# Y-Claw/Multilevel-GNN

Measured on AMD Instinct MI355X. Metric: graphs/sec fwd+bwd, 3-level GNN on 10k-node d=128 synthetic; HBM GB/s %peak, higher is better.
Workload: dtype f32; 1 GPU; configs[1]: ER graphs N=10000 E=160000 x64 per GPU, d=128, 3 GENConv(softmax, res+, LayerNorm) + projection pooling G=25000 k=2 + DiffPool 146->37->10, fp32; step = CSR build (of the next batch, on a second stream) + fwd + bwd + grad all-reduce + Adam; graphs_per_gpu=64, global_batch=64, parallelism=dp1, world_size=1, allreduce_bytes=1429768

## Files before the change

multilevel-gnn_amd/csrc/linear_bwd.hip:

```cpp
#include "split_precision.h"
#include "launch.h"
#include "mlgnn.h"

namespace mlgnn {

constexpr int kLbThreads = 512, kLbWaves = 8, kLbStage = 32;
enum { LB_LN = 0, LB_PLAIN = 1, LB_SHIFT = 2 };

struct LbArgs {
  const float* go; const float* w; const float* x;
  const float* go_parts; const float* x_parts;
  float* dx; float* ws; float* out_parts;
  const float* rstd; const float* gamma; const float* beta;
  const float* lse; float* gt; int* spread;
  int N; int slab_cols;
  int parts_max_with_old;
};

template <int OFF>
__device__ __forceinline__ float lds_read_f32(uint32_t addr) {
  float v;
  asm volatile("ds_read_b32 %0, %1 offset:%2" : "=v"(v) : "v"(addr), "n"(OFF));
  return v;
}
template <int OFF>
__device__ __forceinline__ i32x4 lds_read_b128(uint32_t addr) {
  i32x4 v;
  asm volatile("ds_read_b128 %0, %1 offset:%2" : "=v"(v) : "v"(addr), "n"(OFF));
  return v;
}
template <int OFF>
__device__ __forceinline__ i32x2 lds_read_tr16(uint32_t addr) {
  i32x2 v;
  asm volatile("ds_read_b64_tr_b16 %0, %1 offset:%2" : "=v"(v) : "v"(addr), "n"(OFF));
  return v;
}
#define LB_WAIT_LGKM(N) asm volatile("s_waitcnt lgkmcnt(" #N ")" ::: "memory")
template <int N>
__device__ __forceinline__ void lgkm_landed(i32x4& a, i32x4& b) {
  asm volatile("s_waitcnt lgkmcnt(%2)" : "+v"(a), "+v"(b) : "n"(N) : "memory");
}
template <int N>
__device__ __forceinline__ void lgkm_landed(i32x4& a, i32x4& b, i32x4& c, i32x4& d) {
  asm volatile("s_waitcnt lgkmcnt(%4)" : "+v"(a), "+v"(b), "+v"(c), "+v"(d) : "n"(N) : "memory");
}
template <int N>
__device__ __forceinline__ void lgkm_landed(i32x2& a, i32x2& b, i32x2& c, i32x2& d) {
  asm volatile("s_waitcnt lgkmcnt(%4)" : "+v"(a), "+v"(b), "+v"(c), "+v"(d) : "n"(N) : "memory");
}
template <int N>
__device__ __forceinline__ void lgkm_landed(float (&x)[8]) {
  asm volatile("s_waitcnt lgkmcnt(%8)"
               : "+v"(x[0]), "+v"(x[1]), "+v"(x[2]), "+v"(x[3]), "+v"(x[4]), "+v"(x[5]), "+v"(x[6]), "+v"(x[7])
               : "n"(N) : "memory");
}
template <int N>
__device__ __forceinline__ void lgkm_landed(float (&x)[16]) {
  asm volatile("s_waitcnt lgkmcnt(%16)"
               : "+v"(x[0]), "+v"(x[1]), "+v"(x[2]), "+v"(x[3]), "+v"(x[4]), "+v"(x[5]), "+v"(x[6]), "+v"(x[7]),
                 "+v"(x[8]), "+v"(x[9]), "+v"(x[10]), "+v"(x[11]), "+v"(x[12]), "+v"(x[13]), "+v"(x[14]), "+v"(x[15])
               : "n"(N) : "memory");
}
template <int N>
__device__ __forceinline__ void vm_landed(float (&x)[8]) {
  asm volatile("s_waitcnt vmcnt(%8)"
               : "+v"(x[0]), "+v"(x[1]), "+v"(x[2]), "+v"(x[3]), "+v"(x[4]), "+v"(x[5]), "+v"(x[6]), "+v"(x[7])
               : "n"(N) : "memory");
}
template <int IMM>
__device__ __forceinline__ float glb_load_f32(const void* base, uint32_t byte_off) {
  float v;
  asm volatile("global_load_dword %0, %1, %2 offset:%3" : "=v"(v) : "v"(byte_off), "s"(base), "n"(IMM));
  return v;
}
template <int N>
__device__ __forceinline__ void lb_wait_vm() {
  static_assert(N >= 0 && N <= 63, "vmcnt is a 6-bit counter");
  asm volatile("s_waitcnt vmcnt(%0)" ::"n"(N) : "memory");
}


template <int M, int K, int EPI>
__global__ __launch_bounds__(kLbThreads) void linear_bwd_kernel(const LbArgs p) {
  constexpr int NC = K / 32, NM = kLbWaves / NC, MW = M / NM;
  static_assert(NC * NM == kLbWaves && MW == 128, "instantiated for (M, K) = (128, 256) and (256, 128)");
  static_assert(EPI != LB_LN || NM == 1, "the LayerNorm epilogue needs the whole m range in one wave");
  constexpr int KS = MW / 16;
  constexpr int MT = MW / 32;
  constexpr int GS = M + 4;
  constexpr int kPlaneB = 4 * GS * 16;
  constexpr int kBufB = 2 * kPlaneB;
  constexpr int kXStageB = kLbStage * K * 4;
  constexpr int UPT = M * 4 / kLbThreads;
  constexpr int DMA = kXStageB / 1024 / kLbWaves;
  constexpr int kExB = 2 * kBufB + 3 * kXStageB;
  constexpr int kTotOff = 4 * M + 64;
  constexpr int kExFloats = 4 * M + 64 + (NM == 2 ? kLbWaves * 512 : kLbWaves * 64);
  constexpr int kRsB = kExB + kExFloats * 4;
  extern __shared__ __attribute__((aligned(1024))) unsigned char smem[];
  const uint32_t lds0 = (uint32_t)(uintptr_t)smem;
  float* ex = reinterpret_cast<float*>(smem + kExB);

  const int tid = threadIdx.x;
  const int lane = tid & (kWave - 1);
  const int wave = __builtin_amdgcn_readfirstlane(tid >> 6);
  const int r31 = lane & 31, h = lane >> 5;
  const int c = wave % NC, mh = wave / NC;
  const int col = 32 * c + r31;

  const int n_stages = (p.N + kLbStage - 1) / kLbStage;
  const int s_begin = (int)((int64_t)n_stages * blockIdx.x / gridDim.x);
  const int s_end = (int)((int64_t)n_stages * (blockIdx.x + 1) / gridDim.x);
  const int n = s_end - s_begin;

  float sa, ia, sx, ix, sw, iw;
  pow2_scale(fold_max_parts(p.go_parts), sa, ia);
  pow2_scale(fold_max_parts(p.x_parts), sx, ix);
  {
    float m = 0.f;
    for (int i = tid; i < M * K / 4; i += kLbThreads) {
      const float4 q = reinterpret_cast<const float4*>(p.w)[i];
      m = fmaxf(m, fmaxf(fmaxf(fabsf(q.x), fabsf(q.y)), fmaxf(fabsf(q.z), fabsf(q.w))));
    }
    m = wave_max(m);
    if (lane == 0) ex[wave] = m;
    __syncthreads();
    m = ex[0];
#pragma unroll
    for (int i = 1; i < kLbWaves; ++i) m = fmaxf(m, ex[i]);
    pow2_scale(m, sw, iw);
    __syncthreads();
  }
  auto uniform = [](float v) { return __builtin_bit_cast(float, __builtin_amdgcn_readfirstlane(__builtin_bit_cast(int, v))); };
  sa = uniform(sa); sx = uniform(sx); sw = uniform(sw);
  const float ux = uniform(ia * iw), uw = uniform(ia * ix);

  f16x8 wh[KS], wl[KS];
#pragma unroll
  for (int s = 0; s < KS; ++s) {
    float v[8];
#pragma unroll
    for (int j = 0; j < 8; ++j) v[j] = p.w[(size_t)(mh * MW + 16 * s + 8 * h + j) * K + col];
    split2(v, sw, wh[s], wl[s]);
  }
  float gam = 0.f, bet = 0.f;
  if constexpr (EPI == LB_LN) { gam = p.gamma[col]; bet = p.beta[col]; }
  const bool shift = EPI != LB_SHIFT || p.gt != nullptr;

  auto ucol = [&](int q) { return (tid + q * kLbThreads) % M; };
  auto ubase = [&](int q) { const int G = (tid + q * kLbThreads) / M; return 16 * (G >> 1) + 4 * (G & 1); };
  uint32_t ulds[UPT], goff[UPT];
#pragma unroll
  for (int q = 0; q < UPT; ++q) {
    ulds[q] = (uint32_t)(((tid + q * kLbThreads) / M) * GS + ucol(q)) * 16u;
    goff[q] = (uint32_t)(ubase(q) * M + ucol(q)) * 4u;
  }
  float gr[UPT][8];
  float bsum[UPT];
#pragma unroll
  for (int q = 0; q < UPT; ++q) bsum[q] = 0.f;

  auto row_of = [&](int i) { return (s_begin + min(i, n - 1)) * kLbStage; };
  auto fetch_go = [&](int r0) {
    if (r0 + kLbStage <= p.N) {
      const float* base = p.go + (size_t)r0 * M;
#pragma unroll
      for (int q = 0; q < UPT; ++q) {
        const uint32_t o0 = goff[q], o1 = goff[q] + 8u * M * 4u;
        gr[q][0] = glb_load_f32<0>(base, o0); gr[q][1] = glb_load_f32<M * 4>(base, o0);
        gr[q][2] = glb_load_f32<2 * M * 4>(base, o0); gr[q][3] = glb_load_f32<3 * M * 4>(base, o0);
        gr[q][4] = glb_load_f32<0>(base, o1); gr[q][5] = glb_load_f32<M * 4>(base, o1);
        gr[q][6] = glb_load_f32<2 * M * 4>(base, o1); gr[q][7] = glb_load_f32<3 * M * 4>(base, o1);
      }
    } else {
#pragma unroll
      for (int q = 0; q < UPT; ++q) {
#pragma unroll
        for (int j = 0; j < 8; ++j) {
          const int row = min(r0 + ubase(q) + (j & 3) + 8 * (j >> 2), p.N - 1);
          gr[q][j] = glb_load_f32<0>(p.go, (uint32_t)(row * M + ucol(q)) * 4u);
        }
      }
    }
  };
  auto commit_go = [&](int buf, int r0, bool valid) {
    const bool full = r0 + kLbStage <= p.N;
#pragma unroll
    for (int q = 0; q < UPT; ++q) {
      float v[8];
      float s = 0.f;
#pragma unroll
      for (int j = 0; j < 8; ++j) {
        const bool keep = valid && (full || r0 + ubase(q) + (j & 3) + 8 * (j >> 2) < p.N);
        v[j] = keep ? gr[q][j] : 0.f;
        s += v[j];
      }
      bsum[q] += s;
      f16x8 hi, lo;
      split2(v, sa, hi, lo);
      unsigned char* dst = smem + buf * kBufB + ulds[q];
      *reinterpret_cast<f16x8*>(dst) = hi;
      *reinterpret_cast<f16x8*>(dst + kPlaneB) = lo;
    }
  };
  auto dma_x = [&](int r0, int xbuf) {
#pragma unroll
    for (int i = 0; i < DMA; ++i) {
      const int piece = wave * DMA + i;
      const int e = piece * 256 + lane * 4;
      const int row = min(r0 + e / K, p.N - 1);
      const float* src = p.x + (size_t)row * K + (e % K);
      __builtin_amdgcn_global_load_lds((glb_void_t*)src, (lds_void_t*)(smem + 2 * kBufB + xbuf * kXStageB + piece * 1024), 16, 0, 0);
    }
  };

  f32x16 accw[MT];
#pragma unroll
  for (int t = 0; t < MT; ++t)
#pragma unroll
    for (int r = 0; r < 16; ++r) accw[t][r] = 0.f;
  float dgam = 0.f, dbet = 0.f, om = 0.f, worst = 0.f;

  const uint32_t a_w = lds0 + (uint32_t)((h * GS) + mh * MW + r31) * 16u;
  uint32_t a_tr;
  {
    const int g16 = lane >> 4, b = g16 & 1, hh = g16 >> 1, q = (lane >> 2) & 3, pp = lane & 3;
    a_tr = lds0 + (uint32_t)((2 * b + (pp & 1)) * GS + mh * MW + 8 * hh + q) * 16u + 8u * (uint32_t)(pp >> 1);
  }
  const uint32_t a_x = lds0 + 2 * kBufB + (uint32_t)((4 * h) * K + col) * 4u;

  constexpr int E_L = EPI == LB_LN ? 1 : (EPI == LB_SHIFT ? 8 : 0);
  constexpr int E_S = EPI == LB_SHIFT ? 16 : (EPI == LB_LN ? 16 : 8);
  constexpr int kVmPerIter = E_L + 8 * UPT + DMA + E_S;

  if (n > 0) {
    fetch_go(row_of(0));
    dma_x(row_of(0), 0);
    dma_x(row_of(1), 1);
#pragma unroll
    for (int q = 0; q < UPT; ++q) vm_landed<0>(gr[q]);
    commit_go(0, row_of(0), true);
    __syncthreads();

    for (int i = 0; i < n; ++i) {
      const int r0 = row_of(i);
      const bool full = r0 + kLbStage <= p.N;
      const int buf = i & 1, xbuf = i % 3;
      float lse8[EPI == LB_SHIFT ? 8 : 1];
      if constexpr (EPI == LB_LN) {
        if (lane < 8)
          __builtin_amdgcn_global_load_lds((glb_void_t*)(p.rstd + min(r0 + 4 * lane, (p.N - 1) & ~3)),
                                           (lds_void_t*)(smem + kRsB + ((i % 3) * kLbWaves + wave) * 256), 16, 0, 0);
      }
      if constexpr (EPI == LB_SHIFT) {
        if (!shift) {
#pragma unroll
          for (int q = 0; q < 8; ++q) lse8[q] = glb_load_f32<0>(p.go_parts, 0u);
        } else if (full) {
          const float* base = p.lse + (size_t)r0 * K;
          const uint32_t o0 = (uint32_t)((16 * mh + 4 * h) * K + col) * 4u, o1 = o0 + 8u * K * 4u;
          lse8[0] = glb_load_f32<0>(base, o0); lse8[1] = glb_load_f32<K * 4>(base, o0);
          lse8[2] = glb_load_f32<2 * K * 4>(base, o0); lse8[3] = glb_load_f32<3 * K * 4>(base, o0);
          lse8[4] = glb_load_f32<0>(base, o1); lse8[5] = glb_load_f32<K * 4>(base, o1);
          lse8[6] = glb_load_f32<2 * K * 4>(base, o1); lse8[7] = glb_load_f32<3 * K * 4>(base, o1);
        } else {
#pragma unroll
          for (int q = 0; q < 8; ++q)
            lse8[q] = glb_load_f32<0>(p.lse, (uint32_t)(min(r0 + mfma32_row(8 * mh + q, h), p.N - 1) * K + col) * 4u);
        }
      }
      fetch_go(row_of(i + 1));
      dma_x(row_of(i + 2), (i + 2) % 3);
      __builtin_amdgcn_sched_barrier(0);

      float xv[16];
      {
        const uint32_t ax = a_x + (uint32_t)xbuf * kXStageB;
#define LB_XV(R) xv[R] = lds_read_f32<mfma32_row(R, 0) * K * 4>(ax);
        LB_XV(0) LB_XV(1) LB_XV(2) LB_XV(3) LB_XV(4) LB_XV(5) LB_XV(6) LB_XV(7)
        LB_XV(8) LB_XV(9) LB_XV(10) LB_XV(11) LB_XV(12) LB_XV(13) LB_XV(14) LB_XV(15)
#undef LB_XV
      }
      const uint32_t aw = a_w + (uint32_t)buf * kBufB;
      i32x4 fa[2][2];
      fa[0][0] = lds_read_b128<0>(aw);
      fa[0][1] = lds_read_b128<kPlaneB>(aw);
      lgkm_landed<2>(xv);
#pragma unroll
      for (int kk = 0; kk < 2; ++kk) {
        float v[8];
#pragma unroll
        for (int j = 0; j < 8; ++j) {
          v[j] = xv[8 * kk + j];
          if constexpr (EPI == LB_LN) v[j] = relu_keep_nan(fmaf(v[j], gam, bet));
        }
        f16x8 bh, bl;
        split2(v, sx, bh, bl);
#pragma unroll
        for (int t = 0; t < MT; ++t) {
          const int step = kk * MT + t, slot = step & 1;
          if (step + 1 < 2 * MT) {
            constexpr int kStepB = 2 * GS * 16;
            const int nkk = (step + 1) / MT, nt = (step + 1) % MT;
            if (nkk == 0) {
              if (nt == 1) { fa[1][0] = lds_read_b128<512>(aw); fa[1][1] = lds_read_b128<kPlaneB + 512>(aw); }
              if (nt == 2) { fa[0][0] = lds_read_b128<1024>(aw); fa[0][1] = lds_read_b128<kPlaneB + 1024>(aw); }
              if (nt == 3) { fa[1][0] = lds_read_b128<1536>(aw); fa[1][1] = lds_read_b128<kPlaneB + 1536>(aw); }
            } else {
              if (nt == 0) { fa[0][0] = lds_read_b128<kStepB>(aw); fa[0][1] = lds_read_b128<kPlaneB + kStepB>(aw); }
              if (nt == 1) { fa[1][0] = lds_read_b128<kStepB + 512>(aw); fa[1][1] = lds_read_b128<kPlaneB + kStepB + 512>(aw); }
              if (nt == 2) { fa[0][0] = lds_read_b128<kStepB + 1024>(aw); fa[0][1] = lds_read_b128<kPlaneB + kStepB + 1024>(aw); }
              if (nt == 3) { fa[1][0] = lds_read_b128<kStepB + 1536>(aw); fa[1][1] = lds_read_b128<kPlaneB + kStepB + 1536>(aw); }
            }
            lgkm_landed<2>(fa[slot][0], fa[slot][1]);
          } else {
            lgkm_landed<0>(fa[slot][0], fa[slot][1]);
          }
          const f16x8 ah = __builtin_bit_cast(f16x8, fa[slot][0]), al = __builtin_bit_cast(f16x8, fa[slot][1]);
          f32x16 cw = accw[t];
          cw = __builtin_amdgcn_mfma_f32_32x32x16_f16(al, bh, cw, 0, 0, 0);
          cw = __builtin_amdgcn_mfma_f32_32x32x16_f16(ah, bl, cw, 0, 0, 0);
          cw = __builtin_amdgcn_mfma_f32_32x32x16_f16(ah, bh, cw, 0, 0, 0);
          accw[t] = cw;
        }
      }
      __builtin_amdgcn_sched_barrier(0);
      f32x16 accx;
#pragma unroll
      for (int r = 0; r < 16; ++r) accx[r] = 0.f;
      {
        const uint32_t at = a_tr + (uint32_t)buf * kBufB;
        i32x2 ft[2][4];
#define LB_TR(SLOT, S)                                                                              \
        ft[SLOT][0] = lds_read_tr16<(S) * 256>(at); ft[SLOT][1] = lds_read_tr16<(S) * 256 + 64>(at); \
        ft[SLOT][2] = lds_read_tr16<kPlaneB + (S) * 256>(at); ft[SLOT][3] = lds_read_tr16<kPlaneB + (S) * 256 + 64>(at);
#define LB_DX(SLOT, S)                                                                              \
        {                                                                                           \
          const i32x4 hi4 = {ft[SLOT][0][0], ft[SLOT][0][1], ft[SLOT][1][0], ft[SLOT][1][1]};       \
          const i32x4 lo4 = {ft[SLOT][2][0], ft[SLOT][2][1], ft[SLOT][3][0], ft[SLOT][3][1]};       \
          const f16x8 ah = __builtin_bit_cast(f16x8, hi4), al = __builtin_bit_cast(f16x8, lo4);     \
          accx = __builtin_amdgcn_mfma_f32_32x32x16_f16(al, wh[S], accx, 0, 0, 0);                  \
          accx = __builtin_amdgcn_mfma_f32_32x32x16_f16(ah, wl[S], accx, 0, 0, 0);                  \
          accx = __builtin_amdgcn_mfma_f32_32x32x16_f16(ah, wh[S], accx, 0, 0, 0);                  \
        }
#define LB_LANDED(SLOT, CNT) lgkm_landed<CNT>(ft[SLOT][0], ft[SLOT][1], ft[SLOT][2], ft[SLOT][3]);
        LB_TR(0, 0)
        LB_TR(1, 1) LB_LANDED(0, 4) LB_DX(0, 0)
        LB_TR(0, 2) LB_LANDED(1, 4) LB_DX(1, 1)
        LB_TR(1, 3) LB_LANDED(0, 4) LB_DX(0, 2)
        LB_TR(0, 4) LB_LANDED(1, 4) LB_DX(1, 3)
        LB_TR(1, 5) LB_LANDED(0, 4) LB_DX(0, 4)
        LB_TR(0, 6) LB_LANDED(1, 4) LB_DX(1, 5)
        LB_TR(1, 7) LB_LANDED(0, 4) LB_DX(0, 6)
        LB_LANDED(1, 0) LB_DX(1, 7)
#undef LB_LANDED
#undef LB_TR
#undef LB_DX
      }

      __builtin_amdgcn_sched_barrier(0);
      if constexpr (EPI == LB_LN) {
        float g[16];
        const bool odd_row = (lane & 16) != 0;
        const int r_mine = lane & 15;
        float mine = 0.f;
#pragma unroll
        for (int r = 0; r < 16; ++r) {
          const bool live = full || r0 + mfma32_row(r, h) < p.N;
          const float y = fmaf(xv[r], gam, bet);
          const float gy = (live && y > 0.f) ? accx[r] * ux : 0.f;
          dgam = fmaf(gy, xv[r], dgam);
          dbet += gy;
          g[r] = gy * gam;
          const float gx = g[r] * xv[r];
          const float recv = __builtin_bit_cast(float, __builtin_amdgcn_ds_swizzle(
              __builtin_bit_cast(int, odd_row ? g[r] : gx), 0x401f));
          float u = (odd_row ? gx : g[r]) + recv;
          u += dpp_row_ror<8>(u); u += dpp_row_ror<4>(u); u += dpp_row_ror<2>(u); u += dpp_row_ror<1>(u);
          mine = (r_mine == r) ? u : mine;
        }
        ex[wave * 64 + lane] = mine;
        lb_wait_vm<8 * UPT + DMA>();
        const uint32_t ars = lds0 + kRsB + (uint32_t)(((i % 3) * kLbWaves + wave) * 256 + 16 * h);
        i32x4 rs0_ = lds_read_b128<0>(ars), rs1_ = lds_read_b128<32>(ars), rs2_ = lds_read_b128<64>(ars),
              rs3_ = lds_read_b128<96>(ars);
        lgkm_landed<0>(rs0_, rs1_, rs2_, rs3_);
        float rs[16];
#pragma unroll
        for (int q = 0; q < 4; ++q) {
          rs[q] = __builtin_bit_cast(f32x4, rs0_)[q]; rs[4 + q] = __builtin_bit_cast(f32x4, rs1_)[q];
          rs[8 + q] = __builtin_bit_cast(f32x4, rs2_)[q]; rs[12 + q] = __builtin_bit_cast(f32x4, rs3_)[q];
        }
        __builtin_amdgcn_s_barrier();
        float tot;
        {
          const uint32_t ae = lds0 + kExB + (uint32_t)lane * 4u;
          float e[8] = {lds_read_f32<0>(ae), lds_read_f32<256>(ae), lds_read_f32<512>(ae), lds_read_f32<768>(ae),
                        lds_read_f32<1024>(ae), lds_read_f32<1280>(ae), lds_read_f32<1536>(ae), lds_read_f32<1792>(ae)};
          lgkm_landed<0>(e);
          tot = ((((((e[0] + e[1]) + e[2]) + e[3]) + e[4]) + e[5]) + e[6]) + e[7];
        }
        constexpr float inv_k = 1.0f / K;
#pragma unroll
        for (int r = 0; r < 16; ++r) {
          const float s1 = __shfl(tot, 32 * h + r) * inv_k;
          const float s2 = __shfl(tot, 32 * h + 16 + r) * inv_k;
          g[r] = rs[r] * (g[r] - s1 - xv[r] * s2);
          if (!full && r0 + mfma32_row(r, h) >= p.N) g[r] = 0.f;
          om = fmaxf(om, fabsf(g[r]));
        }
        char* out = reinterpret_cast<char*>(p.dx + (size_t)r0 * K);
        const uint32_t o0 = (uint32_t)(4 * h * K + col) * 4u;
        if (full) {
#pragma unroll
          for (int r = 0; r < 16; ++r)
            *reinterpret_cast<float*>(out + (o0 + (uint32_t)(mfma32_row(r, 0) * K * 4))) = g[r];
        } else {
#pragma unroll
          for (int r = 0; r < 16; ++r)
            if (r0 + mfma32_row(r, h) < p.N)
              *reinterpret_cast<float*>(out + (o0 + (uint32_t)(mfma32_row(r, 0) * K * 4))) = g[r];
        }
      } else {
        float keep[8];
        if constexpr (NM == 2) {
          float* mine = ex + wave * 512 + lane;
#pragma unroll
          for (int q = 0; q < 8; ++q) {
            keep[q] = mh ? accx[8 + q] : accx[q];
            mine[q * 64] = mh ? accx[q] : accx[8 + q];
          }
          LB_WAIT_LGKM(0);
          __builtin_amdgcn_s_barrier();
          const uint32_t ae = lds0 + kExB + (uint32_t)((wave ^ NC) * 512 + lane) * 4u;
          float e[8] = {lds_read_f32<0>(ae), lds_read_f32<256>(ae), lds_read_f32<512>(ae), lds_read_f32<768>(ae),
                        lds_read_f32<1024>(ae), lds_read_f32<1280>(ae), lds_read_f32<1536>(ae), lds_read_f32<1792>(ae)};
          lgkm_landed<0>(e);
#pragma unroll
          for (int q = 0; q < 8; ++q) keep[q] += e[q];
        } else {
#pragma unroll
          for (int q = 0; q < 8; ++q) keep[q] = 0.f;
        }
        if constexpr (EPI == LB_SHIFT) vm_landed<8 * UPT + DMA>(lse8);
        else asm volatile("" : "+v"(keep[0]), "+v"(keep[1]), "+v"(keep[2]), "+v"(keep[3]), "+v"(keep[4]), "+v"(keep[5]),
                          "+v"(keep[6]), "+v"(keep[7])::"memory");
        float v[8], gt[8];
#pragma unroll
        for (int q = 0; q < 8; ++q) {
          v[q] = keep[q] * ux;
          om = fmaxf(om, fabsf(v[q]));
          if constexpr (EPI == LB_SHIFT) {
            gt[q] = v[q] * fast_exp2(-lse8[q]);
            if (shift) worst = fmaxf(worst, fabsf(lse8[q]));
          }
        }
        char* out = reinterpret_cast<char*>(p.dx + (size_t)r0 * K);
        char* out_t = reinterpret_cast<char*>(p.gt + (size_t)r0 * K);
        const uint32_t o0 = (uint32_t)((16 * mh + 4 * h) * K + col) * 4u;
        if (full) {
#pragma unroll
          for (int q = 0; q < 8; ++q)
            *reinterpret_cast<float*>(out + (o0 + (uint32_t)(mfma32_row(q, 0) * K * 4))) = v[q];
          if (EPI == LB_SHIFT && shift) {
#pragma unroll
            for (int q = 0; q < 8; ++q)
              *reinterpret_cast<float*>(out_t + (o0 + (uint32_t)(mfma32_row(q, 0) * K * 4))) = gt[q];
          }
        } else {
#pragma unroll
          for (int q = 0; q < 8; ++q) {
            if (r0 + mfma32_row(8 * mh + q, h) < p.N) {
              const uint32_t o = o0 + (uint32_t)(mfma32_row(q, 0) * K * 4);
              *reinterpret_cast<float*>(out + o) = v[q];
              if (EPI == LB_SHIFT && shift) *reinterpret_cast<float*>(out_t + o) = gt[q];
            }
          }
        }
      }

      __builtin_amdgcn_sched_barrier(0);
      if (full && shift) {
#pragma unroll
        for (int q = 0; q < UPT; ++q) vm_landed<DMA + E_S>(gr[q]);
      } else if (full) {
#pragma unroll
        for (int q = 0; q < UPT; ++q) vm_landed<DMA + (EPI == LB_SHIFT ? 8 : E_S)>(gr[q]);
      } else {
#pragma unroll
        for (int q = 0; q < UPT; ++q) vm_landed<0>(gr[q]);
      }
      commit_go(buf ^ 1, row_of(i + 1), i + 1 < n);
      if (full && shift) lb_wait_vm<kVmPerIter>();
      else if (full) lb_wait_vm<kVmPerIter - (EPI == LB_SHIFT ? 8 : 0)>();
      else lb_wait_vm<0>();
      LB_WAIT_LGKM(0);
      __builtin_amdgcn_s_barrier();
    }
  }
  lb_wait_vm<0>();

  float* slab = p.ws + (size_t)blockIdx.x * p.slab_cols;
#pragma unroll
  for (int t = 0; t < MT; ++t)
#pragma unroll
    for (int r = 0; r < 16; ++r)
      slab[(size_t)(mh * MW + 32 * t + mfma32_row(r, h)) * K + col] = accw[t][r] * uw;
  __syncthreads();
#pragma unroll
  for (int q = 0; q < UPT; ++q) {
    const int u = tid + q * kLbThreads;
    ex[(u / M) * M + ucol(q)] = bsum[q];
  }
  if constexpr (EPI == LB_LN) {
    dgam += __shfl_xor(dgam, 32);
    dbet += __shfl_xor(dbet, 32);
    if (h == 0) { slab[M * K + M + col] = dgam; slab[M * K + M + K + col] = dbet; }
  }
#pragma unroll
  for (int off = 32; off > 0; off >>= 1) { om = fmaxf(om, __shfl_xor(om, off)); worst = fmaxf(worst, __shfl_xor(worst, off)); }
  if (lane == 0) ex[4 * M + wave] = om;
  __syncthreads();
  for (int m = tid; m < M; m += kLbThreads) slab[M * K + m] = (ex[m] + ex[M + m]) + (ex[2 * M + m] + ex[3 * M + m]);
  if (tid == 0 && p.out_parts) {
    float m = ex[4 * M];
#pragma unroll
    for (int i = 1; i < kLbWaves; ++i) m = fmaxf(m, ex[4 * M + i]);
    p.out_parts[blockIdx.x] = p.parts_max_with_old ? fmaxf(m, p.out_parts[blockIdx.x]) : m;
  }
  if constexpr (EPI == LB_SHIFT) {
    if (shift && lane == 0 && worst > kMaxLse) *p.spread = 1;
  }
}

__global__ __launch_bounds__(256) void lb_rowmax_parts_kernel(const float* __restrict__ a, float* __restrict__ pa,
                                                             const float* __restrict__ b, float* __restrict__ pb, int n,
                                                             int* __restrict__ zero4, float* __restrict__ zero_parts) {
  __shared__ float red[2][4];
  if (blockIdx.x == 0 && threadIdx.x < 4 && zero4) zero4[threadIdx.x] = 0;
  if (threadIdx.x == 0 && zero_parts) zero_parts[blockIdx.x] = 0.f;
  const int per = (n + kMaxParts - 1) / kMaxParts;
  const int lo = blockIdx.x * per, hi = min(n, lo + per);
  float ma = 0.f, mb = 0.f;
  for (int i = lo + threadIdx.x; i < hi; i += 256) { if (a) ma = fmaxf(ma, a[i]); if (b) mb = fmaxf(mb, b[i]); }
#pragma unroll
  for (int off = 32; off > 0; off >>= 1) { ma = fmaxf(ma, __shfl_xor(ma, off)); mb = fmaxf(mb, __shfl_xor(mb, off)); }
  if ((threadIdx.x & 63) == 0) { red[0][threadIdx.x >> 6] = ma; red[1][threadIdx.x >> 6] = mb; }
  __syncthreads();
  if (threadIdx.x == 0) {
    if (a) pa[blockIdx.x] = fmaxf(fmaxf(red[0][0], red[0][1]), fmaxf(red[0][2], red[0][3]));
    if (b) pb[blockIdx.x] = fmaxf(fmaxf(red[1][0], red[1][1]), fmaxf(red[1][2], red[1][3]));
  }
}

template <int M, int K>
constexpr int lb_lds_bytes() {
  return 2 * (2 * 4 * (M + 4) * 16) + 3 * (kLbStage * K * 4) + (4 * M + 64) * 4 +
         (M == 256 ? kLbWaves * 512 * 4 : kLbWaves * 64 * 4) +
         3 * kLbWaves * 256;
}

}

using namespace mlgnn;

static bool lb_shape_ok(int64_t N, int64_t M, int64_t K, int epi) {
  if (N <= 0 || N > INT32_MAX - kLbStage) return false;
  if (epi == LB_LN) return M == 128 && K == 256;
  return M == 256 && K == 128;
}

extern "C" int mlgnn_linear_bwd_supported(int64_t N, int64_t M, int64_t K, int epilogue) {
  if (epilogue != LB_LN && epilogue != LB_PLAIN && epilogue != LB_SHIFT) return 0;
  return lb_shape_ok(N, M, K, epilogue) ? 1 : 0;
}

extern "C" int64_t mlgnn_linear_bwd_workspace_floats(int64_t N, int64_t M, int64_t K, int epilogue) {
  if (!mlgnn_linear_bwd_supported(N, M, K, epilogue)) return MLGNN_E_SHAPE;
  const int64_t cols = M * K + M + (epilogue == LB_LN ? 2 * K : 0);
  return (int64_t)kMaxParts * cols + 3 * kMaxParts;
}

extern "C" int mlgnn_linear_bwd(const float* go, const float* w, const float* x, const float* go_max, int go_max_is_parts,
                                const float* x_row_max, int epilogue, const float* rstd, const float* gamma,
                                const float* beta, const float* lse, float* dx, float* grad_shifted,
                                int32_t* shift_flag, float* grad_w_b, float* dx_max_parts, float* workspace,
                                int64_t workspace_floats, int64_t N, int64_t M, int64_t K, void* stream) {
  if (epilogue != LB_LN && epilogue != LB_PLAIN && epilogue != LB_SHIFT) return MLGNN_E_MODE;
  if (!lb_shape_ok(N, M, K, epilogue)) return MLGNN_E_SHAPE;
  if (!go || !w || !x || !go_max || !x_row_max || !dx || !grad_w_b || !workspace) return MLGNN_E_NULL;
  if (epilogue == LB_LN && (!rstd || !gamma || !beta)) return MLGNN_E_NULL;
  if (epilogue == LB_SHIFT && (!lse || !grad_shifted || !shift_flag)) return MLGNN_E_NULL;
  if (workspace_floats < mlgnn_linear_bwd_workspace_floats(N, M, K, epilogue)) return MLGNN_E_WORKSPACE;
  if (!aligned(go, w, x, rstd)) return MLGNN_E_ALIGN;
  hipStream_t s = as_stream(stream);
  const int cols = (int)(M * K + M + (epilogue == LB_LN ? 2 * K : 0));
  float* parts = workspace + (int64_t)kMaxParts * cols;
  const int64_t stages = (N + kLbStage - 1) / kLbStage;
  const int grid = (int)(stages < kMaxParts ? stages : kMaxParts);
  hipLaunchKernelGGL(lb_rowmax_parts_kernel, dim3(kMaxParts), dim3(256), 0, s, go_max_is_parts ? nullptr : go_max, parts,
                     x_row_max, parts + kMaxParts, (int)N, epilogue == LB_SHIFT ? shift_flag : nullptr,
                     (dx_max_parts && grid < kMaxParts) ? dx_max_parts : nullptr);
  int err;
  LbArgs a;
  a.w = w; a.go_parts = go_max_is_parts ? go_max : parts; a.x_parts = parts + kMaxParts;
  a.ws = workspace; a.out_parts = dx_max_parts;
  a.gamma = gamma; a.beta = beta;
  a.spread = shift_flag;
  a.slab_cols = cols;
  const auto launch = [&](auto kernel, int lds_bytes, int grid) {
    if (const hipError_t e = allow_dynamic_lds(kernel, lds_bytes); e != hipSuccess) return (int)e;
    hipLaunchKernelGGL(kernel, dim3(grid), dim3(kLbThreads), lds_bytes, s, a);
    return (int)hipGetLastError();
  };
  if (epilogue == LB_PLAIN) { lse = nullptr; grad_shifted = nullptr; a.spread = nullptr; }
  const int64_t slab_rows = dense_slab_rows(M > K ? M : K);
  for (int64_t r0 = 0; r0 < N; r0 += slab_rows) {
    const int64_t n = N - r0 < slab_rows ? N - r0 : slab_rows;
    const int64_t st = (n + kLbStage - 1) / kLbStage;
    const int grid = (int)(st < kMaxParts ? st : kMaxParts);
    a.go = go + r0 * M; a.x = x + r0 * K; a.dx = dx + r0 * K;
    a.rstd = rstd ? rstd + r0 : nullptr;
    a.lse = lse ? lse + r0 * K : nullptr; a.gt = grad_shifted ? grad_shifted + r0 * K : nullptr;
    a.N = (int)n; a.parts_max_with_old = r0 > 0;
    err = epilogue == LB_LN ? launch(&linear_bwd_kernel<128, 256, LB_LN>, lb_lds_bytes<128, 256>(), grid)
                            : launch(&linear_bwd_kernel<256, 128, LB_SHIFT>, lb_lds_bytes<256, 128>(), grid);
    if (err) return err;
    launch_reduce_partials(workspace, grad_w_b, grid, cols, s, r0 > 0);
  }
  return (int)hipGetLastError();
}
```

Before: 5481 graphs/s.

## Double-buffer LDS exchange area to drop end-of-iteration barrier in linear backward

The cross-wave exchange area in LDS is double-buffered by iteration parity. This lets the trailing vmcnt/lgkmcnt wait and s_barrier at the end of each stage loop be removed, and the commit of the next go tile moves ahead of the epilogue. In the LayerNorm epilogue, the per-row totals are now written back to LDS and read with pipelined ds_read_b64 together with rstd, replacing 32 cross-lane shuffles. The cost is more LDS per block and subtler ordering guarantees between iterations, which rely on the remaining mid-epilogue barrier.

```diff
diff --git a/multilevel-gnn_amd/csrc/linear_bwd.hip b/multilevel-gnn_amd/csrc/linear_bwd.hip
--- a/multilevel-gnn_amd/csrc/linear_bwd.hip
+++ b/multilevel-gnn_amd/csrc/linear_bwd.hip
@@ -4,6 +4,7 @@
 
 namespace mlgnn {
 
+using f32x2 = __attribute__((ext_vector_type(2))) float;
 constexpr int kLbThreads = 512, kLbWaves = 8, kLbStage = 32;
 enum { LB_LN = 0, LB_PLAIN = 1, LB_SHIFT = 2 };
 
@@ -30,19 +31,28 @@
   return v;
 }
 template <int OFF>
+__device__ __forceinline__ i32x2 lds_read_b64(uint32_t addr) {
+  i32x2 v;
+  asm volatile("ds_read_b64 %0, %1 offset:%2" : "=v"(v) : "v"(addr), "n"(OFF));
+  return v;
+}
+template <int OFF>
 __device__ __forceinline__ i32x2 lds_read_tr16(uint32_t addr) {
   i32x2 v;
   asm volatile("ds_read_b64_tr_b16 %0, %1 offset:%2" : "=v"(v) : "v"(addr), "n"(OFF));
   return v;
 }
+__device__ __forceinline__ void lds_write_f32(uint32_t addr, float v) {
+  asm volatile("ds_write_b32 %0, %1" ::"v"(addr), "v"(v) : "memory");
+}
 #define LB_WAIT_LGKM(N) asm volatile("s_waitcnt lgkmcnt(" #N ")" ::: "memory")
 template <int N>
 __device__ __forceinline__ void lgkm_landed(i32x4& a, i32x4& b) {
   asm volatile("s_waitcnt lgkmcnt(%2)" : "+v"(a), "+v"(b) : "n"(N) : "memory");
 }
 template <int N>
-__device__ __forceinline__ void lgkm_landed(i32x4& a, i32x4& b, i32x4& c, i32x4& d) {
-  asm volatile("s_waitcnt lgkmcnt(%4)" : "+v"(a), "+v"(b), "+v"(c), "+v"(d) : "n"(N) : "memory");
+__device__ __forceinline__ void lgkm_landed(i32x2& a, i32x2& b, i32x2& c) {
+  asm volatile("s_waitcnt lgkmcnt(%3)" : "+v"(a), "+v"(b), "+v"(c) : "n"(N) : "memory");
 }
 template <int N>
 __device__ __forceinline__ void lgkm_landed(i32x2& a, i32x2& b, i32x2& c, i32x2& d) {
@@ -79,6 +89,15 @@
   asm volatile("s_waitcnt vmcnt(%0)" ::"n"(N) : "memory");
 }
 
+
+template <int M>
+constexpr int lb_exchange_floats() { return kLbWaves * (M == 256 ? 512 : 64); }
+template <int M, int K>
+constexpr int lb_lds_bytes() {
+  return 2 * (2 * 4 * (M + 4) * 16) + 3 * (kLbStage * K * 4) + 2 * lb_exchange_floats<M>() * 4 +
+         (M == 256 ? 0 : 3 * kLbWaves * 256);
+}
+static_assert(lb_lds_bytes<128, 256>() <= 160 * 1024 && lb_lds_bytes<256, 128>() <= 160 * 1024, "160 KiB of LDS per CU");
 
 template <int M, int K, int EPI>
 __global__ __launch_bounds__(kLbThreads) void linear_bwd_kernel(const LbArgs p) {
@@ -94,9 +113,11 @@
   constexpr int UPT = M * 4 / kLbThreads;
   constexpr int DMA = kXStageB / 1024 / kLbWaves;
   constexpr int kExB = 2 * kBufB + 3 * kXStageB;
-  constexpr int kTotOff = 4 * M + 64;
-  constexpr int kExFloats = 4 * M + 64 + (NM == 2 ? kLbWaves * 512 : kLbWaves * 64);
+  constexpr int kParFloats = lb_exchange_floats<M>();
+  constexpr int kExFloats = 2 * kParFloats;
+  static_assert(kExFloats >= 4 * M + kLbWaves, "the tail of the kernel folds the bias sums and the maxima in this area");
   constexpr int kRsB = kExB + kExFloats * 4;
+  static_assert(kRsB + (EPI == LB_LN ? 3 * kLbWaves * 256 : 0) == lb_lds_bytes<M, K>(), "lb_lds_bytes() is this layout");
   extern __shared__ __attribute__((aligned(1024))) unsigned char smem[];
   const uint32_t lds0 = (uint32_t)(uintptr_t)smem;
   float* ex = reinterpret_cast<float*>(smem + kExB);
@@ -229,9 +250,6 @@
   }
   const uint32_t a_x = lds0 + 2 * kBufB + (uint32_t)((4 * h) * K + col) * 4u;
 
-  constexpr int E_L = EPI == LB_LN ? 1 : (EPI == LB_SHIFT ? 8 : 0);
-  constexpr int E_S = EPI == LB_SHIFT ? 16 : (EPI == LB_LN ? 16 : 8);
-  constexpr int kVmPerIter = E_L + 8 * UPT + DMA + E_S;
 
   if (n > 0) {
     fetch_go(row_of(0));
@@ -359,6 +377,12 @@
       }
 
       __builtin_amdgcn_sched_barrier(0);
+      if constexpr (EPI == LB_SHIFT) vm_landed<DMA>(lse8);
+#pragma unroll
+      for (int q = 0; q < UPT; ++q) vm_landed<DMA>(gr[q]);
+      commit_go(buf ^ 1, row_of(i + 1), i + 1 < n);
+      __builtin_amdgcn_sched_barrier(0);
+      float* expar = ex + buf * kParFloats;
       if constexpr (EPI == LB_LN) {
         float g[16];
         const bool odd_row = (lane & 16) != 0;
@@ -379,36 +403,47 @@
           u += dpp_row_ror<8>(u); u += dpp_row_ror<4>(u); u += dpp_row_ror<2>(u); u += dpp_row_ror<1>(u);
           mine = (r_mine == r) ? u : mine;
         }
-        ex[wave * 64 + lane] = mine;
-        lb_wait_vm<8 * UPT + DMA>();
-        const uint32_t ars = lds0 + kRsB + (uint32_t)(((i % 3) * kLbWaves + wave) * 256 + 16 * h);
-        i32x4 rs0_ = lds_read_b128<0>(ars), rs1_ = lds_read_b128<32>(ars), rs2_ = lds_read_b128<64>(ars),
-              rs3_ = lds_read_b128<96>(ars);
-        lgkm_landed<0>(rs0_, rs1_, rs2_, rs3_);
-        float rs[16];
-#pragma unroll
-        for (int q = 0; q < 4; ++q) {
-          rs[q] = __builtin_bit_cast(f32x4, rs0_)[q]; rs[4 + q] = __builtin_bit_cast(f32x4, rs1_)[q];
-          rs[8 + q] = __builtin_bit_cast(f32x4, rs2_)[q]; rs[12 + q] = __builtin_bit_cast(f32x4, rs3_)[q];
-        }
+        expar[wave * 64 + lane] = mine;
+        LB_WAIT_LGKM(0);
         __builtin_amdgcn_s_barrier();
         float tot;
         {
-          const uint32_t ae = lds0 + kExB + (uint32_t)lane * 4u;
+          const uint32_t ae = lds0 + kExB + (uint32_t)(buf * kParFloats + lane) * 4u;
           float e[8] = {lds_read_f32<0>(ae), lds_read_f32<256>(ae), lds_read_f32<512>(ae), lds_read_f32<768>(ae),
                         lds_read_f32<1024>(ae), lds_read_f32<1280>(ae), lds_read_f32<1536>(ae), lds_read_f32<1792>(ae)};
           lgkm_landed<0>(e);
           tot = ((((((e[0] + e[1]) + e[2]) + e[3]) + e[4]) + e[5]) + e[6]) + e[7];
         }
+        const uint32_t slot = lds0 + kExB + (uint32_t)((buf ^ 1) * kParFloats + wave * 64) * 4u;
+        lds_write_f32(slot + (uint32_t)lane * 4u, tot);
+        const uint32_t as = slot + 128u * (uint32_t)h;
+        const uint32_t ars = lds0 + kRsB + (uint32_t)(((i % 3) * kLbWaves + wave) * 256 + 16 * h);
         constexpr float inv_k = 1.0f / K;
-#pragma unroll
-        for (int r = 0; r < 16; ++r) {
-          const float s1 = __shfl(tot, 32 * h + r) * inv_k;
-          const float s2 = __shfl(tot, 32 * h + 16 + r) * inv_k;
-          g[r] = rs[r] * (g[r] - s1 - xv[r] * s2);
-          if (!full && r0 + mfma32_row(r, h) >= p.N) g[r] = 0.f;
-          om = fmaxf(om, fabsf(g[r]));
-        }
+        i32x2 tp[2][3];
+#define LB_TOT_READ(SLOT, P)                                                                           \
+        tp[SLOT][0] = lds_read_b64<8 * (P)>(as); tp[SLOT][1] = lds_read_b64<64 + 8 * (P)>(as);         \
+        tp[SLOT][2] = lds_read_b64<32 * ((P) >> 1) + 8 * ((P) & 1)>(ars);
+#define LB_TOT_USE(SLOT, P, CNT)                                                                       \
+        lgkm_landed<CNT>(tp[SLOT][0], tp[SLOT][1], tp[SLOT][2]);                                       \
+        _Pragma("unroll") for (int j = 0; j < 2; ++j) {                                                \
+          const int r = 2 * (P) + j;                                                                   \
+          const float s1 = __builtin_bit_cast(f32x2, tp[SLOT][0])[j] * inv_k;                          \
+          const float s2 = __builtin_bit_cast(f32x2, tp[SLOT][1])[j] * inv_k;                          \
+          g[r] = __builtin_bit_cast(f32x2, tp[SLOT][2])[j] * (g[r] - s1 - xv[r] * s2);                 \
+          if (!full && r0 + mfma32_row(r, h) >= p.N) g[r] = 0.f;  \
+          om = fmaxf(om, fabsf(g[r]));                                                                 \
+        }
+        LB_TOT_READ(0, 0)
+        LB_TOT_READ(1, 1) LB_TOT_USE(0, 0, 3)
+        LB_TOT_READ(0, 2) LB_TOT_USE(1, 1, 3)
+        LB_TOT_READ(1, 3) LB_TOT_USE(0, 2, 3)
+        LB_TOT_READ(0, 4) LB_TOT_USE(1, 3, 3)
+        LB_TOT_READ(1, 5) LB_TOT_USE(0, 4, 3)
+        LB_TOT_READ(0, 6) LB_TOT_USE(1, 5, 3)
+        LB_TOT_READ(1, 7) LB_TOT_USE(0, 6, 3)
+        LB_TOT_USE(1, 7, 0)
+#undef LB_TOT_READ
+#undef LB_TOT_USE
         char* out = reinterpret_cast<char*>(p.dx + (size_t)r0 * K);
         const uint32_t o0 = (uint32_t)(4 * h * K + col) * 4u;
         if (full) {
@@ -424,7 +459,7 @@
       } else {
         float keep[8];
         if constexpr (NM == 2) {
-          float* mine = ex + wave * 512 + lane;
+          float* mine = expar + wave * 512 + lane;
 #pragma unroll
           for (int q = 0; q < 8; ++q) {
             keep[q] = mh ? accx[8 + q] : accx[q];
@@ -432,7 +467,7 @@
           }
           LB_WAIT_LGKM(0);
           __builtin_amdgcn_s_barrier();
-          const uint32_t ae = lds0 + kExB + (uint32_t)((wave ^ NC) * 512 + lane) * 4u;
+          const uint32_t ae = lds0 + kExB + (uint32_t)(buf * kParFloats + (wave ^ NC) * 512 + lane) * 4u;
           float e[8] = {lds_read_f32<0>(ae), lds_read_f32<256>(ae), lds_read_f32<512>(ae), lds_read_f32<768>(ae),
                         lds_read_f32<1024>(ae), lds_read_f32<1280>(ae), lds_read_f32<1536>(ae), lds_read_f32<1792>(ae)};
           lgkm_landed<0>(e);
@@ -442,9 +477,6 @@
 #pragma unroll
           for (int q = 0; q < 8; ++q) keep[q] = 0.f;
         }
-        if constexpr (EPI == LB_SHIFT) vm_landed<8 * UPT + DMA>(lse8);
-        else asm volatile("" : "+v"(keep[0]), "+v"(keep[1]), "+v"(keep[2]), "+v"(keep[3]), "+v"(keep[4]), "+v"(keep[5]),
-                          "+v"(keep[6]), "+v"(keep[7])::"memory");
         float v[8], gt[8];
 #pragma unroll
         for (int q = 0; q < 8; ++q) {
@@ -480,22 +512,6 @@
       }
 
       __builtin_amdgcn_sched_barrier(0);
-      if (full && shift) {
-#pragma unroll
-        for (int q = 0; q < UPT; ++q) vm_landed<DMA + E_S>(gr[q]);
-      } else if (full) {
-#pragma unroll
-        for (int q = 0; q < UPT; ++q) vm_landed<DMA + (EPI == LB_SHIFT ? 8 : E_S)>(gr[q]);
-      } else {
-#pragma unroll
-        for (int q = 0; q < UPT; ++q) vm_landed<0>(gr[q]);
-      }
-      commit_go(buf ^ 1, row_of(i + 1), i + 1 < n);
-      if (full && shift) lb_wait_vm<kVmPerIter>();
-      else if (full) lb_wait_vm<kVmPerIter - (EPI == LB_SHIFT ? 8 : 0)>();
-      else lb_wait_vm<0>();
-      LB_WAIT_LGKM(0);
-      __builtin_amdgcn_s_barrier();
     }
   }
   lb_wait_vm<0>();
@@ -551,13 +567,6 @@
     if (a) pa[blockIdx.x] = fmaxf(fmaxf(red[0][0], red[0][1]), fmaxf(red[0][2], red[0][3]));
     if (b) pb[blockIdx.x] = fmaxf(fmaxf(red[1][0], red[1][1]), fmaxf(red[1][2], red[1][3]));
   }
-}
-
-template <int M, int K>
-constexpr int lb_lds_bytes() {
-  return 2 * (2 * 4 * (M + 4) * 16) + 3 * (kLbStage * K * 4) + (4 * M + 64) * 4 +
-         (M == 256 ? kLbWaves * 512 * 4 : kLbWaves * 64 * 4) +
-         3 * kLbWaves * 256;
 }
 
 }
```

Result: faster. 5540 graphs/s, median of 6 (+1.1%).
